# line/open-universe

Measured on AMD Instinct MI355X. Metric: real_time_factor (audio s / wall s), UNIVERSE++ 16 kHz 8-step enhance, higher is better.
Workload: dtype f32; 1 GPU; UNIVERSE++ 16 kHz, 8 diffusion steps, batch=1 utterance(s) of 4 s per GPU per step; network=PP16, n_diffusion_steps=8, batch_per_gpu=1, samples_per_utterance=64000, launches_per_enhance=414

## Files before the change

### include/ouniverse.h

```cpp
#ifndef OUNIVERSE_H
#define OUNIVERSE_H

#include <stddef.h>
#include <stdint.h>

#ifdef __cplusplus
extern "C" {
#endif

#define OU_ABI_VERSION 7

enum {
  OU_OK = 0,
  OU_EINVAL = -1,
  OU_ENOTIMPL = -2,
  OU_EMISSING = -3,
  OU_ESHAPE = -4,
  OU_EHIP = -5,
  OU_ENOMEM = -6,
  OU_ESYNC = -7
};

enum { OU_KIND_UNIVERSE = 0, OU_KIND_UNIVERSE_GAN = 1 };
enum { OU_ACT_NONE = 0, OU_ACT_PRELU = 1, OU_ACT_SNAKE = 2 };
// ... 146 lines not shown
int ou_set_lanes(ou_handle* h, int32_t lanes, int32_t lane);

int ou_set_lane_batch(ou_handle* h, int32_t max_batch);

int ou_lane_capacity(const ou_handle* h, int32_t max_batch);

int ou_check_device_status(ou_handle* h, void* ws);

int ou_set_option(ou_handle* h, const char* key, double value);
int ou_get_option(const ou_handle* h, const char* key, double* value);
int ou_reset_options(ou_handle* h);
int ou_option_count(void);
const char* ou_option_name(int32_t index);
const char* ou_option_doc(int32_t index);
double ou_option_default(int32_t index);

const char* ou_plan_json(const ou_handle* h);
const char* ou_packer_plan_json(const ou_packer* p);
int ou_tensor(const ou_handle* h, const char* name, size_t* byte_offset, int32_t* C, int32_t* T);
int ou_launch_stats(const ou_handle* h, int32_t* n_launches, int32_t* n_conv_launches);
const char* ou_flac_last_error(void);
int ou_flac_info(const uint8_t* data, size_t bytes, int32_t* sample_rate, int32_t* channels, int32_t* bits_per_sample,
                 int64_t* total_samples, uint8_t* md5 );
int ou_flac_decode(const uint8_t* data, size_t bytes, int32_t* out, int64_t capacity_per_channel, int64_t* decoded);


#ifdef __cplusplus
}
#endif
#endif
// ... 1 lines not shown
```

### open-universe_amd/_lib.py

```python
import ctypes
import os
from ctypes import (POINTER, Structure, byref, c_char_p, c_double, c_float, c_int32, c_int64, c_size_t, c_uint32, c_uint64,
                    c_void_p)

OU_MAX_RATES = 8
OU_ABI_VERSION = 7
OU_OK, OU_EINVAL, OU_ENOTIMPL, OU_EMISSING, OU_ESHAPE, OU_EHIP, OU_ENOMEM, OU_ESYNC = 0, -1, -2, -3, -4, -5, -6, -7
OU_KIND_UNIVERSE, OU_KIND_UNIVERSE_GAN = 0, 1
OU_ACT_NONE, OU_ACT_PRELU, OU_ACT_SNAKE = 0, 1, 2
OU_ENH_KEEP_RMS, OU_ENH_USE_AUX_SIGNAL, OU_ENH_NO_PEAK_GUARD, OU_ENH_SERIAL = 1, 2, 4, 8
OU_MAX_ENSEMBLE = 32
OU_ENS_MEAN, OU_ENS_MEDIAN, OU_ENS_SIGNAL_MEDIAN = 0, 1, 2
ENSEMBLE_STATS = {"mean": OU_ENS_MEAN, "median": OU_ENS_MEDIAN, "signal_median": OU_ENS_SIGNAL_MEDIAN}


class NetConfig(Structure):
    _fields_ = [
        ("n_rates", c_int32),
        ("rate_factors", c_int32 * OU_MAX_RATES),
        ("n_channels", c_int32),
        ("fb_kernel_size", c_int32),
        ("n_rff", c_int32),
        ("noise_cond_dim", c_int32),
        ("extra_conv_block", c_int32),
# ... 99 lines not shown
        "ou_noise_fill": (i32, [vp, c_int64, c_int64, i32, POINTER(c_uint64), POINTER(c_int64), POINTER(c_int64), c_uint64,
                                i32, vp]),
        "ou_resample_plan": (i32, [i32, i32, POINTER(i32), POINTER(i32), POINTER(i32), POINTER(i32), POINTER(sz)]),
        "ou_resample_table": (i32, [i32, i32, vp, sz]),
        "ou_resample_length": (c_int64, [i32, i32, c_int64]),
        "ou_resample_tile": (i32, [i32, i32]),
        "ou_resample": (i32, [vp, c_int64, POINTER(c_int64), vp, c_int64, c_int64, i32, i32, i32, vp, sz, vp]),
        "ou_check_device_status": (i32, [vp, vp]),
        "ou_set_option": (i32, [vp, c_char_p, c_double]),
        "ou_get_option": (i32, [vp, c_char_p, POINTER(c_double)]),
        "ou_reset_options": (i32, [vp]),
        "ou_option_count": (i32, []),
        "ou_option_name": (c_char_p, [i32]),
        "ou_option_doc": (c_char_p, [i32]),
        "ou_option_default": (c_double, [i32]),
        "ou_set_stamp_layer": (i32, [vp, c_char_p]),
        "ou_plan_json": (c_char_p, [vp]),
        "ou_packer_plan_json": (c_char_p, [vp]),
        "ou_tensor": (i32, [vp, c_char_p, POINTER(sz), POINTER(i32), POINTER(i32)]),
        "ou_launch_stats": (i32, [vp, POINTER(i32), POINTER(i32)]),
        "ou_workspace_init": (i32, [vp, i32, i32, vp, sz, vp]),
        "ou_sampler_step": (i32, [vp, vp, vp, vp, c_float, c_float, sz, vp]),
        "ou_set_gru_publish_mode": (i32, [vp, i32]),
        "ou_get_gru_publish_mode": (i32, [vp]),
        "ou_set_lanes": (i32, [vp, i32, i32]),
        "ou_set_lane_batch": (i32, [vp, i32]),
        "ou_lane_capacity": (i32, [vp, i32]),
        "ou_transform_frames": (i32, [i32, i32, i32]),
        "ou_transform_forward": (i32, [vp, i32, i32, vp, i32, i32, i32, c_float, c_float, vp, vp]),
        "ou_transform_inverse": (i32, [vp, i32, i32, vp, i32, i32, i32, c_float, c_float, i32, vp, vp, vp]),
# ... 10 lines not shown
        fn.restype = res
        fn.argtypes = args
    _LIB = L
    return L


EXPORTED_SYMBOLS = [
    "ou_version", "ou_last_error", "ou_packer_last_error", "ou_packer_create", "ou_packer_set", "ou_packer_finish",
    "ou_packer_destroy", "ou_packed_bytes", "ou_create", "ou_destroy", "ou_workspace_bytes", "ou_schedule",
    "ou_condition", "ou_score", "ou_aux_to_wav", "ou_enhance", "ou_enhance_var", "ou_check_device_status",
    "ou_segment_plan", "ou_segments_workspace_bytes", "ou_enhance_segments",
    "ou_segment_groups", "ou_segments_var_workspace_bytes", "ou_enhance_segments_var",
    "ou_ensemble_workspace_bytes", "ou_enhance_ensemble", "ou_ensemble_reduce_scratch_bytes", "ou_ensemble_reduce",
    "ou_set_noise_source", "ou_noise_scratch_bytes", "ou_noise_fill",
    "ou_resample_plan", "ou_resample_table", "ou_resample_length", "ou_resample_tile", "ou_resample",
    "ou_set_option", "ou_get_option", "ou_reset_options", "ou_option_count", "ou_option_name", "ou_option_doc", "ou_option_default", "ou_plan_json",
    "ou_packer_plan_json", "ou_tensor", "ou_launch_stats", "ou_workspace_init", "ou_sampler_step",
    "ou_set_gru_publish_mode", "ou_get_gru_publish_mode", "ou_set_lanes", "ou_set_lane_batch", "ou_lane_capacity",
    "ou_transform_frames", "ou_transform_forward", "ou_transform_inverse",
    "ou_flac_last_error", "ou_flac_info", "ou_flac_decode",
]
TUNING_SYMBOLS = ["ou_profile_enable", "ou_profile_read", "ou_profile_read_ticks", "ou_bench_conv", "ou_set_stamp_layer",
]

_EXC = {OU_EINVAL: ValueError, OU_ENOTIMPL: NotImplementedError, OU_EMISSING: KeyError, OU_ESHAPE: ValueError,
        OU_EHIP: RuntimeError, OU_ENOMEM: MemoryError, OU_ESYNC: RuntimeError}


def check(code, handle=None, packer=None):
    if code == OU_OK:
        return
# ... 164 lines not shown
```

### open-universe_amd/csrc/ou_api.cpp

```cpp
#include <hip/hip_runtime.h>

#include <cmath>
#include <cstdio>
#include <cstdlib>
#include <cstring>
#include <map>
#include <string>
#include <vector>

#include "../../include/ouniverse.h"
#include "../../include/ouniverse_tuning.h"
#include "ou_kernels.h"
#include "ou_model.h"

using namespace ou;

namespace {
thread_local std::string g_last_error;
constexpr int kMaxSteps = 256;
constexpr size_t kProfSlots = 32768;
constexpr float kInvSqrt2 = 0.70710678118654752440f;
constexpr size_t align256(size_t bytes) { return (bytes + 255) & ~size_t(255); }

struct TensorRef {
  size_t off;
  int C, T;
};
struct Options {
  int dbg = 0, xcd_map = -1, conv_direct = 5, fuse = -1, fuse_nc = 0, rate_small = 1, fuse_upfir = 1, block3 = 0, d4_fir = 1,
      d4_force = 0, d4_short = 1, d2_wk = 0, wino = 1, d2_map = -1, unfuse64 = 0, preact = 1;
  int gru_v = 2, gru_bmax = 0, gru_ts = 0, gru_upw = 0, gru_backoff = 0, gru_agent = -1, gru_dbg = 0;
  int split = -1;
  int dbg_dec0_under_gru = 0;
  int tile_prefetch = 1;
  int trace = 0, no_overlap = 0, ts = 0, deep_factor = 8, mask_fused = 1, split_wino = 1, d2_tile_rule = 1;
  int ens_share = 1;
  double tile_min = -1.0;
  std::string chain_ts;
};
}

struct ou_packer {
  Model m;
  std::map<std::string, HostTensor> sd;
  std::vector<float> blob;
  std::string err;
};

struct ou_handle {
  Model m;
// ... 60 lines not shown
  const char* key;
  int Options::*ip;
  double Options::*dp;
  bool experiments_only;
  const char* doc;
};
const OptDesc kOptions[] = {
    {"conv_direct", &Options::conv_direct, nullptr, false, "kernel generations the conv launcher may use (0 .. 5, ConvArgs::direct)"},
    {"split", &Options::split, nullptr, false, "-1 rule / 0 never / 1 wherever possible: conv_split_kernel (bf16-split operands)"},
    {"split_wino", &Options::split_wino, nullptr, false, "experiments build: 0 = the plain bf16-split kernel also where its minimal-filtering form would take the layer"},
    {"wino", &Options::wino, nullptr, false, "0: never the minimal-filtering (Winograd / Cook-Toom) kernel variants"},
    {"fuse", &Options::fuse, nullptr, false, "-1 cost model / 0 never / 2 / 3: depth of the fused ConvBlock body (conv_chain kernels)"},
    {"fuse_nc", &Options::fuse_nc, nullptr, false, "128 / 256: columns per tile of the fused ConvBlock body (0: launcher's choice)"},
    {"fuse_upfir", &Options::fuse_upfir, nullptr, false, "0: up-path anti-alias FIR always as its own pass"},
    {"rate_small", &Options::rate_small, nullptr, false, "0: outermost rate-change convs on the generic kernels (no rate_down / rate_up)"},
    {"preact", &Options::preact, nullptr, false, "0: every PReLU in its consumer's operand path (ConvArgs::out_act never set)"},
    {"unfuse64", &Options::unfuse64, nullptr, false, "1: 64-channel ConvBlock bodies as three split-K launches"},
    {"block3", &Options::block3, nullptr, false, "1: the three body convs of a deep-level ConvBlock in one launch (experiments build only)"},
    {"xcd_map", &Options::xcd_map, nullptr, false, "block -> tile mapping of the LDS-tiled conv kernel (-1: launcher's choice)"},
    {"d2_map", &Options::d2_map, nullptr, false, "block -> tile mapping of the wide-load split-K kernels (-1: launcher's choice)"},
    {"d2_tile_rule", &Options::d2_tile_rule, nullptr, false, "0: round 5's 64- vs 32-column rule of the wide-load split-K kernels (ignores that only 64-column tiles have minimal filtering)"},
    {"d2_wk", &Options::d2_wk, nullptr, false, "4 / 8: K slices of conv_direct2_kernel (0: launcher's rule)"},
    {"d4_fir", &Options::d4_fir, nullptr, false, "0: up convs with a fusable FIR stay on the first-generation fused kernel"},
    {"d4_short", &Options::d4_short, nullptr, false, "0: the 401-frame levels at batch 1 stay on the first-generation kernels"},
    {"d4_force", &Options::d4_force, nullptr, false, "10 TM + log2(WK): that conv_direct4 tile shape wherever a layer admits it"},
    {"tile_min", nullptr, &Options::tile_min, false, "wave tiles per SIMD from which the no-split-K kernels take a layer (< 0: 1.2)"},
    {"tile_prefetch", &Options::tile_prefetch, nullptr, false, "0: no LDS prefetch of the epilogue operand in conv_direct3_kernel"},
    {"deep_factor", &Options::deep_factor, nullptr, false, "blocks of 64 x 128 per CU up to which a layer counts as 'deep' (split-K kernels)"},
    {"mask_fused", &Options::mask_fused, nullptr, false, "ragged batches: 0 = a separate tail-mask launch after EVERY producer (reference form of the masks)"},
    {"gru_v", &Options::gru_v, nullptr, false, "2 ring kernel / 1 polling-wave kernel (experiments build)"},
// ... 5 lines not shown
    {"gru_ts", &Options::gru_ts, nullptr, false, "1: per-wave cycle stamps of the GRU kernel into the end of the workspace (tuning)"},
    {"ts", &Options::ts, nullptr, false, "1: per-wave phase stamps in ou_bench_conv (tuning)"},
    {"trace", &Options::trace, nullptr, false, "1: one line per conv launch on stderr"},
    {"no_overlap", &Options::no_overlap, nullptr, false, "1: no side streams inside a call (every kernel alone on the device)"},
    {"ens_share", &Options::ens_share, nullptr, false, "ou_enhance_ensemble: 1 = conditioner once over the B inputs, its results replicated; 0 = over all E * B rows"},
    {"dbg", &Options::dbg, nullptr, true, "phase ablation switches of the conv kernels: WRONG results by design"},
    {"dbg_dec0", &Options::dbg_dec0_under_gru, nullptr, true, "first decoder block under the GRU: upper-bound measurement, WRONG results"},
};
constexpr int kNumOptions = (int)(sizeof(kOptions) / sizeof(kOptions[0]));
const OptDesc* find_option(const char* key) {
  for (int i = 0; i < kNumOptions; i++)
    if (std::strcmp(kOptions[i].key, key) == 0) return &kOptions[i];
  return nullptr;
}
using EnvCfg = Options;

struct Runner {
  ou_handle* h;
  EnvCfg env;
  char* base;
  size_t cap;
  size_t off = 0;
  bool dry;
  hipStream_t st;
  int B;
  hipError_t herr = hipSuccess;
  bool oom = false;
  const char* where = "";
  size_t max_plane = 0;
  bool mel_scale_preset = false;
// ... 216 lines not shown
    return best;
  }

  BlockOut block(const BlockL& Bk, const Tensor& hin, const std::string& nm, const float* film, int film_bs,
                 const float* input_cond, const float* res, bool need_c1 = false, const Tensor* c1_dst = nullptr,
                 const Tensor* v_dst = nullptr) {
    Tensor hu = hin;
    bool small_up = false;
    if (Bk.dir == 2 && (Bk.rc.fir_mode == 0 || Bk.rc.fir_mode == 2)) {
      ConvArgs probe;
      probe.up = Bk.rc.up; probe.stride = Bk.rc.stride; probe.KW = Bk.rc.KW; probe.pad = Bk.rc.pad; probe.Tin = hin.T;
      probe.Nq = hin.T; probe.Tout = hin.T * Bk.rc.up; probe.M = Bk.rc.M; probe.Cout = Bk.rc.Cout; probe.Cin = Bk.rc.Cin;
      probe.fir = Bk.rc.fir_mode == 2 ? h->W : nullptr; probe.fir_len = Bk.rc.fir_len;
      small_up = env.rate_small != 0 && rate_up_supported(probe);
    }
    if (small_up) {
      Epi e;
      e.rate_up = true;
      e.res = res; e.res_scale = kInvSqrt2;
      if (Bk.rc.fir_mode == 2) { e.fir = W(Bk.rc.fir_off); e.fir_len = Bk.rc.fir_len; e.fir_bias = W(Bk.rc.fbias_off); }
      hu = conv(Bk.rc, hin, nm + ".up", e);
    } else if (Bk.dir == 2) {
      if (Bk.rc.fir_mode == 2) {
        Tensor u = alloc(nm + ".upc", Bk.rc.Cout, hin.T * Bk.rc.up);
        hu = alloc(nm + ".up", u.C, u.T);
        if (!dry && ok()) {
          const bool fuse = env.fuse_upfir != 0;
          bool done = false;
          if (fuse) {
            Epi e;
            e.res = res; e.res_scale = kInvSqrt2;
// ... 27 lines not shown
    auto chain_conv = [&](const ConvL& L) {
      ChainConv c;
      c.w = W(L.w_off); c.bias = W(L.b_off); c.alpha = h->alphas[L.a_off]; c.KW = L.KW; c.CK = L.CK;
      if (L.KWP) c.wu = W(L.wu_off);
      return c;
    };
    const int depth = dry ? 0 : plan_chain(Bk, hu.T);

    if (depth == 3 || depth == 2) {
      if (depth == 2) conv(Bk.c1, hu, nm + ".c1", e1, &c1);
      if (ok()) {
        ChainArgs ca;
        ca.depth = depth; ca.B = B; ca.C = Bk.C; ca.T = hu.T; ca.Mp = Bk.c1.Mp;
        ca.x = depth == 3 ? hu.p : c1.p;
        ca.y = v.p; ca.res = hu.p; ca.res_scale = kInvSqrt2;
        if (depth == 3) {
          ca.add = e1.add; ca.add_scale = e1.add_scale; ca.film = e1.film; ca.film_bstride = e1.film_bstride;
          ca.c1_out = need_c1 ? c1.p : nullptr;
          ca.cv[0] = chain_conv(Bk.c1); ca.cv[1] = chain_conv(Bk.c2); ca.cv[2] = chain_conv(Bk.c3);
        } else {
          ca.cv[0] = chain_conv(Bk.c2); ca.cv[1] = chain_conv(Bk.c3);
        }
        ca.force_nc = h->fuse_nc;
        ca.wino = env.wino && env.conv_direct >= 5;
        ca.lens = lens_of(hu.T);
        if (!env.chain_ts.empty() && nm == env.chain_ts) ca.tstamps = (long long*)(base + cap - (16u << 20));
        int variant = -1;
        if (h->profile && h->prof_dev && h->prof_used < kProfSlots) {
          ou_handle::ProfRec rec;
          rec.flops = 0;
          double wbytes = 0;
          for (int s2 = 0; s2 < depth; s2++) {
            rec.flops += 2.0 * Bk.C * (double)hu.T * Bk.C * ca.cv[s2].KW * B;
            wbytes += 4.0 * Bk.C * Bk.C * ca.cv[s2].KW;
          }
          rec.bytes = 4.0 * B * (double)Bk.C * hu.T * (2 + (depth == 2 ? 1 : 0) + (ca.add ? 1 : 0)) + wbytes;
          rec.cfg = -1;
          ca.prof = h->prof_dev + 32 * h->prof_used;
          h->prof.push_back(rec);
          h->prof_used++;
        }
        chk(launch_chain(ca, h->num_cu, st, &variant), nm.c_str());
        if (ca.prof) h->prof.back().cfg = variant;
        if (h->trace)
          std::fprintf(stderr, "OU_TRACE chain %-63s variant=%d depth=%d C=%d T=%d B=%d\n", nm.c_str(), variant, depth,
                       Bk.C, hu.T, B);
        h->n_conv++;
      }
    } else {
      Epi e3;
      e3.res = hu.p; e3.res_scale = kInvSqrt2;
// ... 420 lines not shown
  for (int i = 0; i < kNumOptions; i++) {
    const OptDesc& d = kOptions[i];
    char buf[96];
    if (d.ip) std::snprintf(buf, sizeof buf, "%s\"%s\": %d", i ? ", " : "", d.key, h->opt.*(d.ip));
    else std::snprintf(buf, sizeof buf, "%s\"%s\": %.9g", i ? ", " : "", d.key, h->opt.*(d.dp));
    o += buf;
  }
  o += "}";
  o += std::string(", \"noise_source\": \"") + (h->noise_src.on ? "counter" : "tensor") + "\"";
  const std::string& j = h->m.json;
  const size_t close = j.rfind('}');
  h->plan_with_options = close == std::string::npos ? "{" + o + "}" : j.substr(0, close) + ", " + o + j.substr(close);
  return h->plan_with_options.c_str();
}

int ou_set_option(ou_handle* h, const char* key, double value) {
  if (!h || !key) return fail(h, OU_EINVAL, "bad argument");
  const OptDesc* d = find_option(key);
  if (!d) return fail(h, OU_EMISSING, std::string("ou_set_option: no such option: ") + key);
#ifndef OU_EXPERIMENTS
  if (d->experiments_only && value != 0.0)
    return fail(h, OU_ENOTIMPL, std::string("ou_set_option: `") + key + "` makes calls return wrong results by design and exists in "
                "the experiments build (make EXPERIMENTS=1) only");
#endif
  if (d->ip) {
    if (value != std::floor(value) || std::fabs(value) > 2e9) return fail(h, OU_EINVAL, std::string("ou_set_option: `") + key + "` takes an integer");
    h->opt.*(d->ip) = (int)value;
  } else {
    h->opt.*(d->dp) = value;
  }
  h->trace = h->opt.trace != 0;
  h->overlap = h->opt.no_overlap == 0;
  return OU_OK;
}

int ou_get_option(const ou_handle* h, const char* key, double* value) {
  if (!h || !key || !value) return fail(const_cast<ou_handle*>(h), OU_EINVAL, "bad argument");
  const OptDesc* d = find_option(key);
  if (!d) return fail(const_cast<ou_handle*>(h), OU_EMISSING, std::string("ou_get_option: no such option: ") + key);
  *value = d->ip ? (double)(h->opt.*(d->ip)) : h->opt.*(d->dp);
  return OU_OK;
}

int ou_reset_options(ou_handle* h) {
  if (!h) return fail(h, OU_EINVAL, "bad argument");
  const std::string keep = h->opt.chain_ts;
  h->opt = Options();
  h->opt.chain_ts = keep;
// ... 1551 lines not shown
```

### open-universe_amd/csrc/ou_conv_chain.hip

```cpp
#include "ou_kernels.h"
#include "ou_internal.h"
#include "ou_dev.h"

#include <cmath>
#include <cstdlib>
#include <type_traits>

namespace ou {

#ifdef OU_EXPERIMENTS
template <int MT, int NWV>
__global__ __launch_bounds__(64 * NWV) void conv_chain_kernel(ChainArgs p, int TN, int ntiles) {
  constexpr int C = 32 * MT, NTN = NWV / MT, NC = 32 * NTN, XS = NC + 4, NTH = 64 * NWV;
  constexpr int WSLOT = 96 * C;
  constexpr int MAXW = (WSLOT / 4 + NTH - 1) / NTH;
  constexpr int RPW = C / NWV, NCG = NC / 64;
  constexpr int U = 4;
  static_assert(NC % 64 == 0 && RPW * 4 <= 64 && C % NWV == 0, "input tile mapping");
  extern __shared__ __attribute__((aligned(16))) float smem[];
  float* bufA = smem;
  float* bufB = bufA + C * XS;
  float* Wb = bufB + C * XS;
  float* prm = Wb + 2 * WSLOT;

// ... 207 lines not shown
  };
  run_stage(S0{});
  run_stage(S1{});
  if (D == 3) run_stage(S2{});

  if (ts_on && lane == 0) {
    long long* o = p.tstamps + ((size_t)blockIdx.x * NWV + wave) * 8;
    o[0] = tsv[1] - tsv[0]; o[1] = tsv[2] - tsv[1]; o[2] = t_mma; o[3] = t_epi; o[4] = t_bar;
    o[5] = __builtin_readcyclecounter() - tsv[0]; o[6] = t_iss; o[7] = t_ws;
  }
  if (p.prof && tid == 0) atomicMin(p.prof + 16 + (blockIdx.x & 15), ~(unsigned long long)__builtin_amdgcn_s_memrealtime());
}

#endif

template <int MT, bool D3>
__global__ __launch_bounds__(256) void conv_chainw_kernel(ChainArgs p, int TN, int ntiles) {
  constexpr int C = 32 * MT, NW = 4, NWN = NW / MT, NC = 64 * NWN, XS = NC + 8, NTH = 64 * NW, NS = D3 ? 3 : 2;
  constexpr int WI = C * C / NTH;
  static_assert(!D3 || MT == 1, "depth 3: the 32-channel level");
  extern __shared__ __attribute__((aligned(16))) float smem[];
  float* bufB = smem;
  float* bufA = bufB + C * XS;
  float* Ua0 = bufA + (D3 ? C * XS : 0);
  float* Ub0 = Ua0 + C * C * 4;
  float* U2 = Ub0 + (D3 ? C * C * 2 : 0);
  float* U3 = U2 + (D3 ? C * C * 4 : 0);
  float* prm = D3 ? U3 + C * C * 4 : Ub0;

  const int tid = threadIdx.x, lane = tid & 63;
  const int wave = __builtin_amdgcn_readfirstlane(tid >> 6);
  const int wm = wave % MT, wn = wave / MT;
  const int lhalf = lane >> 5, l31 = lane & 31;
  const int tile = blockIdx.x % ntiles, b = blockIdx.x / ntiles;
  const int T = p.T, Mp = p.Mp;
  const int rlen = ragged_len(p.lens, b), Tl = rlen < T ? rlen : T;
  if (p.prof && tid == 0) atomicMin(p.prof + (blockIdx.x & 15), (unsigned long long)__builtin_amdgcn_s_memrealtime());
  const int t0 = tile * TN;
  constexpr int KW0 = D3 ? 5 : 3, PAD0 = (KW0 - 1) / 2, R0 = D3 ? 2 : 1;
  const bool ts_on = p.tstamps != nullptr;
  long long tsv[9] = {0, 0, 0, 0, 0, 0, 0, 0, 0};
  if (ts_on) tsv[0] = __builtin_readcyclecounter();
  const size_t rowbase = (size_t)b * C * T;
// ... 10 lines not shown
      wa[k] = *reinterpret_cast<const f32x4*>(s1);
      wa2[k] = *reinterpret_cast<const f32x2*>(s1 + 4);
      wb[k] = *reinterpret_cast<const f32x4*>(p.cv[1].wu + ((size_t)ci * Mp + m) * 4);
      wc[k] = *reinterpret_cast<const f32x4*>(p.cv[2].wu + ((size_t)ci * Mp + m) * 4);
    } else {
      wa[k] = *reinterpret_cast<const f32x4*>(p.cv[0].wu + ((size_t)ci * Mp + m) * 4);
    }
  }
  const int pcol = 64 * wn + 2 * l31;
  const int tw = t0 - R0 - PAD0 + pcol;
  const int sh = tw < 0 ? -tw : 0;
  unsigned wmask = 0;
#pragma unroll
  for (int i = 0; i <= KW0; i++) wmask |= (tw + i >= 0 && tw + i < T) ? (1u << i) : 0u;
  const bool edge = __builtin_amdgcn_readfirstlane((t0 - R0 - PAD0 < 0 || t0 - R0 - PAD0 + NC + KW0 - 1 > T) ? 1 : 0) != 0;
  f32x4 gw4[C / 2];
  f32x2 gw2[D3 ? C / 2 : 1];
  {
    const __amdgpu_buffer_rsrc_t rx = make_rsrc(p.x + rowbase, plane);
    const int wvo = wmask ? (lhalf * T + tw + sh) * 4 : (int)0x80000000;
#pragma unroll
    for (int I = 0; I < C / 2; I++) {
      gw4[I] = __builtin_bit_cast(f32x4, __builtin_amdgcn_raw_buffer_load_b128(rx, wvo, 2 * I * Tb, 0));
      if constexpr (D3) gw2[I] = __builtin_bit_cast(f32x2, __builtin_amdgcn_raw_buffer_load_b64(rx, wvo + 16, 2 * I * Tb, 0));
    }
  }
  if constexpr (!D3) {
#pragma unroll
    for (int k = 0; k < WI; k++) {
      const int it = tid + k * NTH, ci = it / C, m = it % C;
      wb[k] = *reinterpret_cast<const f32x4*>(p.cv[1].wu + ((size_t)ci * Mp + m) * 4);
    }
  }
  if (ts_on) tsv[1] = __builtin_readcyclecounter();
  for (int i = tid; i < C; i += NTH) {
    prm[i] = p.cv[0].bias[i];
    prm[C + i] = p.cv[1].bias[i];
    prm[2 * C + i] = D3 ? p.cv[2].bias[i] : 0.f;
    prm[3 * C + i] = (D3 && p.film) ? p.film[(size_t)b * p.film_bstride + i] : 1.f;
    prm[4 * C + i] = (D3 && p.film) ? p.film[(size_t)b * p.film_bstride + C + i] : 0.f;
  }
  for (int i = tid; i < C * 8; i += NTH) {
    bufB[(i >> 3) * XS + NC + (i & 7)] = 0.f;
    if constexpr (D3) bufA[(i >> 3) * XS + NC + (i & 7)] = 0.f;
  }
#pragma unroll
  for (int k = 0; k < WI; k++) {
    const int it = tid + k * NTH;
    *reinterpret_cast<f32x4*>(&Ua0[it * 4]) = wa[k];
    if constexpr (D3) *reinterpret_cast<f32x2*>(&Ub0[it * 2]) = wa2[k];
  }
  __syncthreads();
  if (ts_on) tsv[2] = __builtin_readcyclecounter();

  const int lrow = 32 * wm + 4 * lhalf;

  auto run_stage = [&](auto SC) {
    constexpr int s = decltype(SC)::value;
    constexpr int KW = (D3 && s == 0) ? 5 : 3, NX = KW + 1;
    constexpr bool last = s == NS - 1;
    constexpr bool first3 = D3 && s == 0;
    const float* inb = (s == 1) ? bufB : bufA;
    float* outb = (s == 0) ? bufB : bufA;
    const float* Ua = D3 ? (s == 0 ? Ua0 : (s == 1 ? U2 : U3)) : Ua0;
    constexpr int Rs = NS - 1 - s;
    const int t = t0 - Rs + pcol;
    const bool in0 = t >= 0 && t < Tl, in1 = t + 1 >= 0 && t + 1 < Tl;
    const bool on0 = t >= 0 && t < T, on1 = t + 1 >= 0 && t + 1 < T;
    f32x2 ev[16];
    const float* src = last ? p.res : (first3 ? p.add : nullptr);
    if (src) {
      const __amdgpu_buffer_rsrc_t rs = make_rsrc(src + rowbase, plane);
      const int vo = (on0 || on1) ? (lrow * T + t) * 4 : (int)0x80000000;
#pragma unroll
      for (int r = 0; r < 16; r++)
        ev[r] = __builtin_bit_cast(f32x2, __builtin_amdgcn_raw_buffer_load_b64(rs, vo, ((r & 3) + 8 * (r >> 2)) * Tb, 0));
    }
    floatx16 acc[NX];
#pragma unroll
    for (int x = 0; x < NX; x++)
#pragma unroll
      for (int r = 0; r < 16; r++) acc[x][r] = 0.f;
    const float* ap = Ua + (lhalf * C + 32 * wm + l31) * 4;
    const float* ap2 = Ub0 + (lhalf * C + 32 * wm + l31) * 2;
    const float* bp = inb + lhalf * XS + pcol;
    struct Ops { f32x4 a4; f32x2 a2, d01, d23; };
    auto fetch = [&](int I) {
      Ops o;
      o.a4 = *reinterpret_cast<const f32x4*>(ap + I * (2 * C * 4));
      o.a2 = f32x2{0.f, 0.f}; o.d01 = f32x2{0.f, 0.f}; o.d23 = f32x2{0.f, 0.f};
      if constexpr (KW == 5) o.a2 = *reinterpret_cast<const f32x2*>(ap2 + I * (2 * C * 2));
      if constexpr (s > 0) {
        const float* bq = bp + I * (2 * XS);
        o.d01 = *reinterpret_cast<const f32x2*>(bq);
        o.d23 = *reinterpret_cast<const f32x2*>(bq + 2);
      }
      return o;
    };
    auto transform = [&](const Ops& o, int I, float (&V)[NX]) {
      float X[6] = {o.d01.x, o.d01.y, o.d23.x, o.d23.y, 0.f, 0.f};
      if constexpr (s == 0) {
        const float L[6] = {gw4[I].x, gw4[I].y, gw4[I].z, gw4[I].w, D3 ? gw2[D3 ? I : 0].x : 0.f, D3 ? gw2[D3 ? I : 0].y : 0.f};
        const float a0 = p.cv[0].alpha;
        if (edge) {
#pragma unroll
          for (int i = 0; i < NX; i++) {
            float v = L[i];
            v = sh == 1 ? (i >= 1 ? L[i >= 1 ? i - 1 : 0] : 0.f) : v;
            v = sh == 2 ? (i >= 2 ? L[i >= 2 ? i - 2 : 0] : 0.f) : v;
            v = sh == 4 ? (i >= 4 ? L[i >= 4 ? i - 4 : 0] : 0.f) : v;
            X[i] = ((wmask >> i) & 1u) ? v : 0.f;
          }
        } else {
#pragma unroll
          for (int i = 0; i < NX; i++) X[i] = L[i];
        }
#pragma unroll
// ... 79 lines not shown
        const int kr = (r & 3) + 8 * (r >> 2);
        float a = in0 ? v0[r] : 0.f;
        float c = in1 ? v1[r] : 0.f;
        a = a >= 0.f ? a : an * a;
        c = c >= 0.f ? c : an * c;
        *reinterpret_cast<f32x2*>(&out_l[kr * XS]) = f32x2{a, c};
      }
    } else {
      const __amdgpu_buffer_rsrc_t ry = make_rsrc(p.y + rowbase, plane);
      const bool st0 = on0 && pcol < TN, st1 = on1 && pcol + 1 < TN;
      const int vo = (st0 && st1) ? (lrow * T + t) * 4 : (int)0x80000000;
#pragma unroll
      for (int r = 0; r < 16; r++) {
        const int kr = (r & 3) + 8 * (r >> 2);
        float v0 = o0[r] + bias_l[kr], v1 = o1[r] + bias_l[kr];
        if (p.res) { v0 = (v0 + ev[r].x) * p.res_scale; v1 = (v1 + ev[r].y) * p.res_scale; }
        v0 = in0 ? v0 : 0.f; v1 = in1 ? v1 : 0.f;
        __builtin_amdgcn_raw_buffer_store_b64(__builtin_bit_cast(u32x2, f32x2{v0, v1}), ry, vo, kr * Tb, 0);
      }
    }
    if constexpr (D3 && s == 0) {
#pragma unroll
      for (int k = 0; k < WI; k++) {
        const int it = tid + k * NTH;
        *reinterpret_cast<f32x4*>(&U2[it * 4]) = wb[k];
        *reinterpret_cast<f32x4*>(&U3[it * 4]) = wc[D3 ? k : 0];
      }
    }
    if constexpr (!D3 && s == 0) {
      __syncthreads();
#pragma unroll
// ... 1 lines not shown
    }
    if constexpr (!last) __syncthreads();
    if (ts_on) tsv[4 + 2 * s] = __builtin_readcyclecounter();
  };
  run_stage(std::integral_constant<int, 0>{});
  run_stage(std::integral_constant<int, 1>{});
  if constexpr (D3) run_stage(std::integral_constant<int, 2>{});
  if (ts_on && lane == 0) {
    long long* o = p.tstamps + ((size_t)blockIdx.x * NW + wave) * 8;
#pragma unroll
    for (int i = 0; i < 8; i++) o[i] = tsv[i + 1] - tsv[i];
  }
  if (p.prof && tid == 0) atomicMin(p.prof + 16 + (blockIdx.x & 15), ~(unsigned long long)__builtin_amdgcn_s_memrealtime());
}
static constexpr size_t kChainwSmem32 = 4 * ((size_t)2 * 32 * (256 + 8) + 32 * 32 * (4 + 2 + 4 + 4) + 5 * 32);
static constexpr size_t kChainwSmem64 = 4 * ((size_t)64 * (128 + 8) + 64 * 64 * 4 + 5 * 64);
static int chainw_kind(const ChainArgs& a) {
  if (!a.wino || a.T % 4 || (long)a.C * a.T * 4 >= (1L << 31) || a.force_nc != 0) return 0;
  if (a.C == 32 && a.depth == 3 && a.cv[0].KW == 5 && a.cv[1].KW == 3 && a.cv[2].KW == 3 && a.cv[0].wu && a.cv[1].wu && a.cv[2].wu &&
      a.T >= 252)
    return 1;
  if (a.C == 64 && a.depth == 2 && a.cv[0].KW == 3 && a.cv[1].KW == 3 && a.cv[0].wu && a.cv[1].wu && a.T >= 126 && !a.add &&
      !a.film && !a.c1_out)
    return 2;
  return 0;
}

struct ChainVariant {
  int C, NC, NWV;
  void (*kern)(ChainArgs, int, int);
// ... 52 lines not shown
  double best = -1.0;
  for (int i = 0; i < kNumChainVariants; i++) {
    const ChainVariant& v = kChainVariants[i];
    if (v.C != a.C || (a.force_nc && v.NC != a.force_nc)) continue;
    const double c = chain_variant_cost(a, v, num_cu);
    if (best < 0 || c < best) { best = c; if (nc_out) *nc_out = v.NC; }
  }
  return best;
}

hipError_t init_chain_kernels() {
  {
    hipError_t e = hipFuncSetAttribute(reinterpret_cast<const void*>(conv_chainw_kernel<1, true>),
                                       hipFuncAttributeMaxDynamicSharedMemorySize, (int)kChainwSmem32);
    if (e != hipSuccess) return e;
    e = hipFuncSetAttribute(reinterpret_cast<const void*>(conv_chainw_kernel<2, false>), hipFuncAttributeMaxDynamicSharedMemorySize,
                            (int)kChainwSmem64);
    if (e != hipSuccess) return e;
  }
  for (int i = 0; i < kNumChainVariants; i++) {
    hipError_t e = hipFuncSetAttribute(reinterpret_cast<const void*>(kChainVariants[i].kern),
                                       hipFuncAttributeMaxDynamicSharedMemorySize, (int)chain_smem_bytes(kChainVariants[i]));
    if (e != hipSuccess) return e;
  }
  return hipSuccess;
}

hipError_t launch_chain(const ChainArgs& a, int num_cu, hipStream_t st, int* variant) {
  int nc = 0;
  if (chain_cost(a, num_cu, &nc) < 0) return hipErrorInvalidConfiguration;
  if (const int kind = chainw_kind(a)) {
    const int TN = kind == 1 ? 252 : 126, ntiles = (a.T + TN - 1) / TN;
    if (variant) *variant = 190 + a.depth;
    if (kind == 1) hipLaunchKernelGGL((conv_chainw_kernel<1, true>), dim3(ntiles * a.B), dim3(256), kChainwSmem32, st, a, TN, ntiles);
    else hipLaunchKernelGGL((conv_chainw_kernel<2, false>), dim3(ntiles * a.B), dim3(256), kChainwSmem64, st, a, TN, ntiles);
    return hipGetLastError();
  }
  for (int i = 0; i < kNumChainVariants; i++) {
    const ChainVariant& v = kChainVariants[i];
    if (v.C != a.C || v.NC != nc) continue;
    int R0 = 0;
    for (int s = 1; s < a.depth; s++) R0 += (a.cv[s].KW - 1) / 2;
    const int TN = v.NC - 2 * R0;
    const int ntiles = (a.T + TN - 1) / TN;
    if (variant) *variant = 100 + 10 * a.depth + i;
    hipLaunchKernelGGL(v.kern, dim3(ntiles * a.B), dim3(64 * v.NWV), chain_smem_bytes(v), st, a, TN, ntiles);
    return hipGetLastError();
  }
  return hipErrorInvalidConfiguration;
// ... 299 lines not shown
```

### open-universe_amd/csrc/ou_kernels.h

```cpp
#pragma once
#include <hip/hip_runtime.h>

#include <cstddef>
#include <cstdint>

namespace ou {

struct ConvArgs {
  const float* x = nullptr;
  const float* w = nullptr;
  const float* wd = nullptr;
  const float* wu = nullptr;
  const void* wsplit = nullptr;
  const void* wsplitw = nullptr;
  int split_wino = 1;
  const float* bias = nullptr;
  float* y = nullptr;
  const float* in_scale = nullptr;
  int act = 0;
  float alpha_val = 0.f;
  const float* add = nullptr;
  const float* film = nullptr;
  const float* res = nullptr;
  float add_scale = 1.f, res_scale = 1.f;
// ... 181 lines not shown
  const float* x = nullptr;
  float* y = nullptr;
  const float* res = nullptr;
  float res_scale = 1.f;
  const float* add = nullptr;
  float add_scale = 1.f;
  const float* film = nullptr;
  int film_bstride = 0;
  float* c1_out = nullptr;
  int B = 1, C = 32, T = 0, Mp = 64;
  int depth = 3;
  ChainConv cv[3];
  int force_nc = 0;
  int wino = 1;
  const int* lens = nullptr;
  unsigned long long* prof = nullptr;
  long long* tstamps = nullptr;
};
double chain_cost(const ChainArgs& a, int num_cu, int* nc_out);
hipError_t launch_chain(const ChainArgs& a, int num_cu, hipStream_t st, int* variant);
hipError_t launch_conv_block3(const ConvArgs* cv, unsigned long long* bar, unsigned* err, int num_cu, hipStream_t st,
                              int* cfg_out);

struct GruArgs {
  const float* gx = nullptr;
  const float* whh = nullptr;
  const float* bhn = nullptr;
  float* out = nullptr;
  const float* res = nullptr;
  float res_scale = 1.f;
  unsigned long long* xchg = nullptr;
  unsigned long long* xchg_base = nullptr;
  size_t xchg_granules = 0;
// ... 25 lines not shown
```

Measured before the change: 611.7 x_realtime.

## Fuse outermost up-rate conv and FIR into the 32-channel fused ConvBlock body

Adds a prologue variant of the Winograd chain kernel that computes the outermost rate-up conv (64→32 channels, phase GEMM via MFMA), applies the 5-tap anti-alias FIR, bias and residual, and writes the result into LDS instead of global memory. The body's first conv and final residual then read from that LDS tile. This removes one launch per up block and the global write and read of the upsampled tensor. In exchange it costs extra LDS, which can lower occupancy, and redundant halo recomputation per tile. It is enabled by default via a new fuse_rate option, alongside an option-validation helper.

```diff
diff --git a/include/ouniverse.h b/include/ouniverse.h
--- a/include/ouniverse.h
+++ b/include/ouniverse.h
@@ -184,6 +184,9 @@
 const char* ou_option_name(int32_t index);
 const char* ou_option_doc(int32_t index);
 double ou_option_default(int32_t index);
+int ou_option_check(const char* key, double value);
+int32_t ou_plan_rate_fuse(int32_t fuse_rate, int32_t dir, int32_t C, int32_t rc_Cin, int32_t rc_up, int32_t fir_len, int32_t body_depth,
+                          int32_t body_wino32);
 
 const char* ou_plan_json(const ou_handle* h);
 const char* ou_packer_plan_json(const ou_packer* p);
diff --git a/open-universe_amd/_lib.py b/open-universe_amd/_lib.py
--- a/open-universe_amd/_lib.py
+++ b/open-universe_amd/_lib.py
@@ -137,6 +137,8 @@
         "ou_option_name": (c_char_p, [i32]),
         "ou_option_doc": (c_char_p, [i32]),
         "ou_option_default": (c_double, [i32]),
+        "ou_option_check": (i32, [c_char_p, c_double]),
+        "ou_plan_rate_fuse": (i32, [i32] * 8),
         "ou_set_stamp_layer": (i32, [vp, c_char_p]),
         "ou_plan_json": (c_char_p, [vp]),
         "ou_packer_plan_json": (c_char_p, [vp]),
@@ -177,7 +179,7 @@
     "ou_ensemble_workspace_bytes", "ou_enhance_ensemble", "ou_ensemble_reduce_scratch_bytes", "ou_ensemble_reduce",
     "ou_set_noise_source", "ou_noise_scratch_bytes", "ou_noise_fill",
     "ou_resample_plan", "ou_resample_table", "ou_resample_length", "ou_resample_tile", "ou_resample",
-    "ou_set_option", "ou_get_option", "ou_reset_options", "ou_option_count", "ou_option_name", "ou_option_doc", "ou_option_default", "ou_plan_json",
+    "ou_set_option", "ou_get_option", "ou_reset_options", "ou_option_count", "ou_option_name", "ou_option_doc", "ou_option_default", "ou_option_check", "ou_plan_rate_fuse", "ou_plan_json",
     "ou_packer_plan_json", "ou_tensor", "ou_launch_stats", "ou_workspace_init", "ou_sampler_step",
     "ou_set_gru_publish_mode", "ou_get_gru_publish_mode", "ou_set_lanes", "ou_set_lane_batch", "ou_lane_capacity",
     "ou_transform_frames", "ou_transform_forward", "ou_transform_inverse",
diff --git a/open-universe_amd/csrc/ou_api.cpp b/open-universe_amd/csrc/ou_api.cpp
--- a/open-universe_amd/csrc/ou_api.cpp
+++ b/open-universe_amd/csrc/ou_api.cpp
@@ -34,6 +34,7 @@
   int dbg_dec0_under_gru = 0;
   int tile_prefetch = 1;
   int trace = 0, no_overlap = 0, ts = 0, deep_factor = 8, mask_fused = 1, split_wino = 1, d2_tile_rule = 1;
+  int fuse_rate = 1;
   int ens_share = 1;
   double tile_min = -1.0;
   std::string chain_ts;
@@ -124,6 +125,7 @@
     {"fuse_nc", &Options::fuse_nc, nullptr, false, "128 / 256: columns per tile of the fused ConvBlock body (0: launcher's choice)"},
     {"fuse_upfir", &Options::fuse_upfir, nullptr, false, "0: up-path anti-alias FIR always as its own pass"},
     {"rate_small", &Options::rate_small, nullptr, false, "0: outermost rate-change convs on the generic kernels (no rate_down / rate_up)"},
+    {"fuse_rate", &Options::fuse_rate, nullptr, false, "0: the outermost up conv as a launch of its own (rate_up_kernel), not as the prologue of the fused ConvBlock body (0 .. 1)"},
     {"preact", &Options::preact, nullptr, false, "0: every PReLU in its consumer's operand path (ConvArgs::out_act never set)"},
     {"unfuse64", &Options::unfuse64, nullptr, false, "1: 64-channel ConvBlock bodies as three split-K launches"},
     {"block3", &Options::block3, nullptr, false, "1: the three body convs of a deep-level ConvBlock in one launch (experiments build only)"},
@@ -159,6 +161,13 @@
   return nullptr;
 }
 using EnvCfg = Options;
+
+int plan_rate_fuse(int fuse_rate, int dir, int C, int rc_Cin, int rc_up, int fir_len, int body_depth, bool body_wino32) {
+  if (!fuse_rate || dir != 2) return 0;
+  if (C != 32 || rc_Cin != 64 || rc_up != 2 || fir_len != 5) return 0;
+  if (body_depth != 3 || !body_wino32) return 0;
+  return 2;
+}
 
 struct Runner {
   ou_handle* h;
@@ -405,7 +414,25 @@
       probe.fir = Bk.rc.fir_mode == 2 ? h->W : nullptr; probe.fir_len = Bk.rc.fir_len;
       small_up = env.rate_small != 0 && rate_up_supported(probe);
     }
-    if (small_up) {
+    bool up_fused = false;
+    if (small_up && !dry && ok() && Bk.rc.fir_mode == 2) {
+      const int Tb = hin.T * Bk.rc.up;
+      const int depth_b = plan_chain(Bk, Tb);
+      ChainArgs sh;
+      sh.depth = 3; sh.B = B; sh.C = Bk.C; sh.T = Tb; sh.Mp = Bk.c1.Mp; sh.force_nc = h->fuse_nc;
+      sh.cv[0].KW = Bk.c1.KW; sh.cv[1].KW = Bk.c2.KW; sh.cv[2].KW = Bk.c3.KW;
+      if (Bk.c1.KWP) sh.cv[0].wu = h->W;
+      if (Bk.c2.KWP) sh.cv[1].wu = h->W;
+      if (Bk.c3.KWP) sh.cv[2].wu = h->W;
+      sh.wino = env.wino && env.conv_direct >= 5;
+      up_fused = plan_rate_fuse(env.fuse_rate, Bk.dir, Bk.C, Bk.rc.Cin, Bk.rc.up, Bk.rc.fir_len, depth_b,
+                                depth_b == 3 && chain_up_supported(sh)) == 2 && Bk.rc.Cout == Bk.C && Bk.rc.M == 2 * Bk.C;
+    }
+    if (up_fused) {
+      hu = alloc("", Bk.rc.Cout, hin.T * Bk.rc.up);
+      hu.p = nullptr;
+      h->tensors.erase(nm + ".up");
+    } else if (small_up) {
       Epi e;
       e.rate_up = true;
       e.res = res; e.res_scale = kInvSqrt2;
@@ -463,6 +490,13 @@
         ca.depth = depth; ca.B = B; ca.C = Bk.C; ca.T = hu.T; ca.Mp = Bk.c1.Mp;
         ca.x = depth == 3 ? hu.p : c1.p;
         ca.y = v.p; ca.res = hu.p; ca.res_scale = kInvSqrt2;
+        if (up_fused) {
+          if (depth != 3) { herr = hipErrorInvalidConfiguration; where = "fuse_rate: body plan changed"; return BlockOut(); }
+          const ConvL& U = Bk.rc;
+          ca.up_x = hin.p; ca.up_w = W(U.w_off); ca.up_Mp = U.Mp; ca.up_fir = W(U.fir_off); ca.up_bias = W(U.fbias_off);
+          ca.up_res = res; ca.up_res_scale = kInvSqrt2;
+          ca.up_act = U.act ? 1 : 0; ca.up_alpha = U.act ? h->alphas[U.a_off] : 0.f;
+        }
         if (depth == 3) {
           ca.add = e1.add; ca.add_scale = e1.add_scale; ca.film = e1.film; ca.film_bstride = e1.film_bstride;
           ca.c1_out = need_c1 ? c1.p : nullptr;
@@ -484,6 +518,11 @@
             wbytes += 4.0 * Bk.C * Bk.C * ca.cv[s2].KW;
           }
           rec.bytes = 4.0 * B * (double)Bk.C * hu.T * (2 + (depth == 2 ? 1 : 0) + (ca.add ? 1 : 0)) + wbytes;
+          if (up_fused) {
+            const ConvL& U = Bk.rc;
+            rec.flops += 2.0 * U.M * (double)hin.T * U.Cin * U.KW * B;
+            rec.bytes += 4.0 * ((double)B * ((double)U.Cin * hin.T + (double)U.Cout * hu.T) + (double)U.M * U.Cin * U.KW);
+          }
           rec.cfg = -1;
           ca.prof = h->prof_dev + 32 * h->prof_used;
           h->prof.push_back(rec);
@@ -934,6 +973,18 @@
   return h->plan_with_options.c_str();
 }
 
+static const char* option_value_error(const OptDesc* d, double value) {
+  if (!d->ip) return nullptr;
+  if (value != std::floor(value) || std::fabs(value) > 2e9) return "takes an integer";
+  if (d->ip == &Options::fuse_rate && (value < 0 || value > 1)) return "is 0 or 1";
+  return nullptr;
+}
+int ou_option_check(const char* key, double value) {
+  const OptDesc* d = key ? find_option(key) : nullptr;
+  if (!d) return OU_EMISSING;
+  return option_value_error(d, value) ? OU_EINVAL : OU_OK;
+}
+
 int ou_set_option(ou_handle* h, const char* key, double value) {
   if (!h || !key) return fail(h, OU_EINVAL, "bad argument");
   const OptDesc* d = find_option(key);
@@ -944,7 +995,7 @@
                 "the experiments build (make EXPERIMENTS=1) only");
 #endif
   if (d->ip) {
-    if (value != std::floor(value) || std::fabs(value) > 2e9) return fail(h, OU_EINVAL, std::string("ou_set_option: `") + key + "` takes an integer");
+    if (const char* why = option_value_error(d, value)) return fail(h, OU_EINVAL, std::string("ou_set_option: `") + key + "` " + why);
     h->opt.*(d->ip) = (int)value;
   } else {
     h->opt.*(d->dp) = value;
@@ -952,6 +1003,11 @@
   h->trace = h->opt.trace != 0;
   h->overlap = h->opt.no_overlap == 0;
   return OU_OK;
+}
+
+int32_t ou_plan_rate_fuse(int32_t fuse_rate, int32_t dir, int32_t C, int32_t rc_Cin, int32_t rc_up, int32_t fir_len, int32_t body_depth,
+                          int32_t body_wino32) {
+  return plan_rate_fuse(fuse_rate, dir, C, rc_Cin, rc_up, fir_len, body_depth, body_wino32 != 0);
 }
 
 int ou_get_option(const ou_handle* h, const char* key, double* value) {
diff --git a/open-universe_amd/csrc/ou_conv_chain.hip b/open-universe_amd/csrc/ou_conv_chain.hip
--- a/open-universe_amd/csrc/ou_conv_chain.hip
+++ b/open-universe_amd/csrc/ou_conv_chain.hip
@@ -245,11 +245,12 @@
 
 #endif
 
-template <int MT, bool D3>
+template <int MT, bool D3, bool UPF = false>
 __global__ __launch_bounds__(256) void conv_chainw_kernel(ChainArgs p, int TN, int ntiles) {
   constexpr int C = 32 * MT, NW = 4, NWN = NW / MT, NC = 64 * NWN, XS = NC + 8, NTH = 64 * NW, NS = D3 ? 3 : 2;
   constexpr int WI = C * C / NTH;
   static_assert(!D3 || MT == 1, "depth 3: the 32-channel level");
+  static_assert(!UPF || D3, "the up-conv prologue: depth 3 only");
   extern __shared__ __attribute__((aligned(16))) float smem[];
   float* bufB = smem;
   float* bufA = bufB + C * XS;
@@ -258,6 +259,7 @@
   float* U2 = Ub0 + (D3 ? C * C * 2 : 0);
   float* U3 = U2 + (D3 ? C * C * 4 : 0);
   float* prm = D3 ? U3 + C * C * 4 : Ub0;
+  float* hub = prm + 5 * C;
 
   const int tid = threadIdx.x, lane = tid & 63;
   const int wave = __builtin_amdgcn_readfirstlane(tid >> 6);
@@ -298,9 +300,9 @@
 #pragma unroll
   for (int i = 0; i <= KW0; i++) wmask |= (tw + i >= 0 && tw + i < T) ? (1u << i) : 0u;
   const bool edge = __builtin_amdgcn_readfirstlane((t0 - R0 - PAD0 < 0 || t0 - R0 - PAD0 + NC + KW0 - 1 > T) ? 1 : 0) != 0;
-  f32x4 gw4[C / 2];
-  f32x2 gw2[D3 ? C / 2 : 1];
-  {
+  f32x4 gw4[UPF ? 1 : C / 2];
+  f32x2 gw2[(D3 && !UPF) ? C / 2 : 1];
+  if constexpr (!UPF) {
     const __amdgpu_buffer_rsrc_t rx = make_rsrc(p.x + rowbase, plane);
     const int wvo = wmask ? (lhalf * T + tw + sh) * 4 : (int)0x80000000;
 #pragma unroll
@@ -324,9 +326,87 @@
     prm[3 * C + i] = (D3 && p.film) ? p.film[(size_t)b * p.film_bstride + i] : 1.f;
     prm[4 * C + i] = (D3 && p.film) ? p.film[(size_t)b * p.film_bstride + C + i] : 0.f;
   }
-  for (int i = tid; i < C * 8; i += NTH) {
-    bufB[(i >> 3) * XS + NC + (i & 7)] = 0.f;
-    if constexpr (D3) bufA[(i >> 3) * XS + NC + (i & 7)] = 0.f;
+  if constexpr (UPF) {
+    constexpr int UK2 = 32, UPP = 161, NQ = XS / 4 - 1;
+    constexpr int QPT = (C * NQ + NTH - 1) / NTH;
+    float* Us = smem;
+    static_assert(64 * UPP <= 2 * C * XS, "phase-GEMM tile inside the activation tiles");
+    const int Tin = T >> 1, q0 = (t0 >> 1) - 3;
+    const bool ures = p.up_res != nullptr;
+    const __amdgpu_buffer_rsrc_t rr = make_rsrc((ures ? p.up_res : p.y) + rowbase, plane);
+    f32x4 rs4[QPT];
+#pragma unroll
+    for (int k = 0; k < QPT; k++) {
+      const int e = tid + k * NTH, co = e / NQ, j = 4 * (e - co * NQ), t = t0 - 4 + j;
+      const int vo = (ures && e < C * NQ && t >= 0 && t < T) ? (co * T + t) * 4 : (int)0x80000000;
+      rs4[k] = __builtin_bit_cast(f32x4, __builtin_amdgcn_raw_buffer_load_b128(rr, vo, 0, 0));
+    }
+    const int um = wave & 1;
+    const __amdgpu_buffer_rsrc_t rxu = make_rsrc(p.up_x + (size_t)b * 64 * Tin, plane);
+    float ub[3][UK2], ua[UK2];
+    bool uin[3];
+#pragma unroll
+    for (int k = 0; k < 3; k++) {
+      const int un = (wave >> 1) + 2 * k, fq = q0 + 32 * un + l31;
+      uin[k] = un < 5 && fq >= 0 && fq < Tin;
+      const int vo = uin[k] ? (lhalf * Tin + fq) * 4 : (int)0x80000000;
+#pragma unroll
+      for (int ks = 0; ks < UK2; ks++) ub[k][ks] = buf_load(rxu, vo, 2 * ks * Tin * 4);
+    }
+#pragma unroll
+    for (int ks = 0; ks < UK2; ks++) ua[ks] = p.up_w[(size_t)(2 * ks + lhalf) * p.up_Mp + 32 * um + l31];
+    const float ualpha = p.up_alpha;
+    const bool uact = p.up_act != 0;
+#pragma unroll
+    for (int k = 0; k < 3; k++) {
+      const int un = (wave >> 1) + 2 * k;
+      if (un < 5) {
+        floatx16 acc;
+#pragma unroll
+        for (int r = 0; r < 16; r++) acc[r] = 0.f;
+#pragma unroll
+        for (int ks = 0; ks < UK2; ks++) {
+          const float x = ub[k][ks];
+          acc = __builtin_amdgcn_mfma_f32_32x32x2f32(ua[ks], (uact && x < 0.f) ? ualpha * x : x, acc, 0, 0, 0);
+        }
+#pragma unroll
+        for (int r = 0; r < 16; r++) {
+          const int row = 32 * um + (r & 3) + 8 * (r >> 2) + 4 * lhalf;
+          Us[row * UPP + 32 * un + l31] = uin[k] ? acc[r] : 0.f;
+        }
+      }
+    }
+    float uf[5];
+#pragma unroll
+    for (int j = 0; j < 5; j++) uf[j] = p.up_fir[j];
+    __syncthreads();
+#pragma unroll
+    for (int k = 0; k < QPT; k++) {
+      const int e = tid + k * NTH, co = e / NQ, j0 = 4 * (e - co * NQ), t = t0 - 4 + j0;
+      if (e >= C * NQ) continue;
+      const float* urow = Us + (co * 2) * UPP;
+      const float bi = p.up_bias[co];
+      f32x4 o;
+#pragma unroll
+      for (int s4 = 0; s4 < 4; s4++) {
+        int qf = (j0 + s4) >> 1, ph = (j0 + s4) & 1;
+        float v = 0.f;
+#pragma unroll
+        for (int j = 0; j < 5; j++) {
+          v = fmaf(uf[j], urow[ph * UPP + qf], v);
+          if (++ph == 2) { ph = 0; qf++; }
+        }
+        v += bi;
+        if (ures) v = (v + rs4[k][s4]) * p.up_res_scale;
+        o[s4] = (t + s4 >= 0 && t + s4 < Tl) ? v : 0.f;
+      }
+      *reinterpret_cast<f32x4*>(&hub[co * XS + j0]) = o;
+    }
+  } else {
+    for (int i = tid; i < C * 8; i += NTH) {
+      bufB[(i >> 3) * XS + NC + (i & 7)] = 0.f;
+      if constexpr (D3) bufA[(i >> 3) * XS + NC + (i & 7)] = 0.f;
+    }
   }
 #pragma unroll
   for (int k = 0; k < WI; k++) {
@@ -335,6 +415,12 @@
     if constexpr (D3) *reinterpret_cast<f32x2*>(&Ub0[it * 2]) = wa2[k];
   }
   __syncthreads();
+  if constexpr (UPF) {
+    for (int i = tid; i < C * 8; i += NTH) {
+      bufB[(i >> 3) * XS + NC + (i & 7)] = 0.f;
+      bufA[(i >> 3) * XS + NC + (i & 7)] = 0.f;
+    }
+  }
   if (ts_on) tsv[2] = __builtin_readcyclecounter();
 
   const int lrow = 32 * wm + 4 * lhalf;
@@ -344,7 +430,8 @@
     constexpr int KW = (D3 && s == 0) ? 5 : 3, NX = KW + 1;
     constexpr bool last = s == NS - 1;
     constexpr bool first3 = D3 && s == 0;
-    const float* inb = (s == 1) ? bufB : bufA;
+    constexpr bool ldsB = s > 0 || UPF;
+    const float* inb = (s == 1) ? bufB : (s == 0 ? hub : bufA);
     float* outb = (s == 0) ? bufB : bufA;
     const float* Ua = D3 ? (s == 0 ? Ua0 : (s == 1 ? U2 : U3)) : Ua0;
     constexpr int Rs = NS - 1 - s;
@@ -352,7 +439,7 @@
     const bool in0 = t >= 0 && t < Tl, in1 = t + 1 >= 0 && t + 1 < Tl;
     const bool on0 = t >= 0 && t < T, on1 = t + 1 >= 0 && t + 1 < T;
     f32x2 ev[16];
-    const float* src = last ? p.res : (first3 ? p.add : nullptr);
+    const float* src = last ? (UPF ? nullptr : p.res) : (first3 ? p.add : nullptr);
     if (src) {
       const __amdgpu_buffer_rsrc_t rs = make_rsrc(src + rowbase, plane);
       const int vo = (on0 || on1) ? (lrow * T + t) * 4 : (int)0x80000000;
@@ -368,23 +455,29 @@
     const float* ap = Ua + (lhalf * C + 32 * wm + l31) * 4;
     const float* ap2 = Ub0 + (lhalf * C + 32 * wm + l31) * 2;
     const float* bp = inb + lhalf * XS + pcol;
-    struct Ops { f32x4 a4; f32x2 a2, d01, d23; };
+    struct Ops { f32x4 a4; f32x2 a2, d01, d23, d45; };
     auto fetch = [&](int I) {
       Ops o;
       o.a4 = *reinterpret_cast<const f32x4*>(ap + I * (2 * C * 4));
-      o.a2 = f32x2{0.f, 0.f}; o.d01 = f32x2{0.f, 0.f}; o.d23 = f32x2{0.f, 0.f};
+      o.a2 = f32x2{0.f, 0.f}; o.d01 = f32x2{0.f, 0.f}; o.d23 = f32x2{0.f, 0.f}; o.d45 = f32x2{0.f, 0.f};
       if constexpr (KW == 5) o.a2 = *reinterpret_cast<const f32x2*>(ap2 + I * (2 * C * 2));
-      if constexpr (s > 0) {
+      if constexpr (ldsB) {
         const float* bq = bp + I * (2 * XS);
         o.d01 = *reinterpret_cast<const f32x2*>(bq);
         o.d23 = *reinterpret_cast<const f32x2*>(bq + 2);
+        if constexpr (KW == 5) o.d45 = *reinterpret_cast<const f32x2*>(bq + 4);
       }
       return o;
     };
     auto transform = [&](const Ops& o, int I, float (&V)[NX]) {
-      float X[6] = {o.d01.x, o.d01.y, o.d23.x, o.d23.y, 0.f, 0.f};
-      if constexpr (s == 0) {
-        const float L[6] = {gw4[I].x, gw4[I].y, gw4[I].z, gw4[I].w, D3 ? gw2[D3 ? I : 0].x : 0.f, D3 ? gw2[D3 ? I : 0].y : 0.f};
+      float X[6] = {o.d01.x, o.d01.y, o.d23.x, o.d23.y, o.d45.x, o.d45.y};
+      if constexpr (s == 0 && UPF) {
+        const float a0 = p.cv[0].alpha;
+#pragma unroll
+        for (int i = 0; i < NX; i++) X[i] = X[i] >= 0.f ? X[i] : a0 * X[i];
+      } else if constexpr (s == 0) {
+        const float L[6] = {gw4[UPF ? 0 : I].x, gw4[UPF ? 0 : I].y, gw4[UPF ? 0 : I].z, gw4[UPF ? 0 : I].w, D3 ? gw2[(D3 && !UPF) ? I : 0].x : 0.f,
+                            D3 ? gw2[(D3 && !UPF) ? I : 0].y : 0.f};
         const float a0 = p.cv[0].alpha;
         if (edge) {
 #pragma unroll
@@ -494,7 +587,10 @@
       for (int r = 0; r < 16; r++) {
         const int kr = (r & 3) + 8 * (r >> 2);
         float v0 = o0[r] + bias_l[kr], v1 = o1[r] + bias_l[kr];
-        if (p.res) { v0 = (v0 + ev[r].x) * p.res_scale; v1 = (v1 + ev[r].y) * p.res_scale; }
+        if constexpr (UPF) {
+          const f32x2 e = *reinterpret_cast<const f32x2*>(&hub[(lrow + kr) * XS + pcol + 4]);
+          v0 = (v0 + e.x) * p.res_scale; v1 = (v1 + e.y) * p.res_scale;
+        } else if (p.res) { v0 = (v0 + ev[r].x) * p.res_scale; v1 = (v1 + ev[r].y) * p.res_scale; }
         v0 = in0 ? v0 : 0.f; v1 = in1 ? v1 : 0.f;
         __builtin_amdgcn_raw_buffer_store_b64(__builtin_bit_cast(u32x2, f32x2{v0, v1}), ry, vo, kr * Tb, 0);
       }
@@ -526,6 +622,7 @@
   if (p.prof && tid == 0) atomicMin(p.prof + 16 + (blockIdx.x & 15), ~(unsigned long long)__builtin_amdgcn_s_memrealtime());
 }
 static constexpr size_t kChainwSmem32 = 4 * ((size_t)2 * 32 * (256 + 8) + 32 * 32 * (4 + 2 + 4 + 4) + 5 * 32);
+static constexpr size_t kChainwSmem32Up = kChainwSmem32 + 4 * (size_t)32 * (256 + 8);
 static constexpr size_t kChainwSmem64 = 4 * ((size_t)64 * (128 + 8) + 64 * 64 * 4 + 5 * 64);
 static int chainw_kind(const ChainArgs& a) {
   if (!a.wino || a.T % 4 || (long)a.C * a.T * 4 >= (1L << 31) || a.force_nc != 0) return 0;
@@ -608,6 +705,9 @@
     hipError_t e = hipFuncSetAttribute(reinterpret_cast<const void*>(conv_chainw_kernel<1, true>),
                                        hipFuncAttributeMaxDynamicSharedMemorySize, (int)kChainwSmem32);
     if (e != hipSuccess) return e;
+    e = hipFuncSetAttribute(reinterpret_cast<const void*>(conv_chainw_kernel<1, true, true>), hipFuncAttributeMaxDynamicSharedMemorySize,
+                            (int)kChainwSmem32Up);
+    if (e != hipSuccess) return e;
     e = hipFuncSetAttribute(reinterpret_cast<const void*>(conv_chainw_kernel<2, false>), hipFuncAttributeMaxDynamicSharedMemorySize,
                             (int)kChainwSmem64);
     if (e != hipSuccess) return e;
@@ -620,13 +720,22 @@
   return hipSuccess;
 }
 
+static bool chain_up_ok(const ChainArgs& a) {
+  return a.up_x && a.up_w && a.up_fir && a.up_bias && !a.x && !a.res && a.up_Mp >= 64 && a.C == 32 && a.depth == 3;
+}
+bool chain_up_supported(const ChainArgs& a) { return chainw_kind(a) == 1; }
+
 hipError_t launch_chain(const ChainArgs& a, int num_cu, hipStream_t st, int* variant) {
   int nc = 0;
+  if (a.up_x && !kNumChainVariants && chainw_kind(a) != 1) return hipErrorInvalidConfiguration;
   if (chain_cost(a, num_cu, &nc) < 0) return hipErrorInvalidConfiguration;
   if (const int kind = chainw_kind(a)) {
     const int TN = kind == 1 ? 252 : 126, ntiles = (a.T + TN - 1) / TN;
-    if (variant) *variant = 190 + a.depth;
-    if (kind == 1) hipLaunchKernelGGL((conv_chainw_kernel<1, true>), dim3(ntiles * a.B), dim3(256), kChainwSmem32, st, a, TN, ntiles);
+    if (variant) *variant = a.up_x ? kChainVariantUp : 190 + a.depth;
+    if (a.up_x) {
+      if (kind != 1 || !chain_up_ok(a)) return hipErrorInvalidConfiguration;
+      hipLaunchKernelGGL((conv_chainw_kernel<1, true, true>), dim3(ntiles * a.B), dim3(256), kChainwSmem32Up, st, a, TN, ntiles);
+    } else if (kind == 1) hipLaunchKernelGGL((conv_chainw_kernel<1, true>), dim3(ntiles * a.B), dim3(256), kChainwSmem32, st, a, TN, ntiles);
     else hipLaunchKernelGGL((conv_chainw_kernel<2, false>), dim3(ntiles * a.B), dim3(256), kChainwSmem64, st, a, TN, ntiles);
     return hipGetLastError();
   }
diff --git a/open-universe_amd/csrc/ou_kernels.h b/open-universe_amd/csrc/ou_kernels.h
--- a/open-universe_amd/csrc/ou_kernels.h
+++ b/open-universe_amd/csrc/ou_kernels.h
@@ -219,9 +219,18 @@
   int force_nc = 0;
   int wino = 1;
   const int* lens = nullptr;
+  const float* up_x = nullptr;
+  const float* up_w = nullptr;
+  const float* up_fir = nullptr;
+  const float* up_bias = nullptr;
+  const float* up_res = nullptr;
+  float up_res_scale = 1.f, up_alpha = 0.f;
+  int up_act = 0, up_Mp = 64;
   unsigned long long* prof = nullptr;
   long long* tstamps = nullptr;
 };
+constexpr int kChainVariantUp = 183;
+bool chain_up_supported(const ChainArgs& a);
 double chain_cost(const ChainArgs& a, int num_cu, int* nc_out);
 hipError_t launch_chain(const ChainArgs& a, int num_cu, hipStream_t st, int* variant);
 hipError_t launch_conv_block3(const ConvArgs* cv, unsigned long long* bar, unsigned* err, int num_cu, hipStream_t st,
```

Result: slower. 598.2 x_realtime (-2.2%).
